# mike-gimelfarb/bboptpy

Measured on AMD Instinct MI355X. Metric: candidate-evals/sec, higher is better.
Workload: dtype f64; 1 GPU; ActiveCMAES n=128 np=4096 rosenbrock, 256 independent populations per GPU in lockstep; populations_per_gpu=256, n=128, np=4096, objective=rosenbrock

## Files before the change

bboptpy_amd/csrc/bbo_cma.hip:

```cpp
#include "bbo_cma_kernels.hpp"
#include "bbo_sep_kernels.hpp"
#include "bbo_chol_kernels.hpp"
#include "bbo_eig_mw.hpp"

#include <algorithm>
#include <atomic>
#include <cmath>
#include <cstdlib>
#include <limits>

namespace bbo {

namespace {

enum { K_SAMPLE = 0, K_RANK, K_WHITEN, K_GRAM, K_PATHS, K_COV, K_EIGEN, K_POST, K_STOP, K_COUNT };
static const char *const K_NAMES[K_COUNT] = { "bbo:cma_sample_eval", "bbo:cma_rank", "bbo:cma_whiten", "bbo:cma_gram", "bbo:cma_paths", "bbo:cma_cov", "bbo:cma_eigen", "bbo:cma_post", "bbo:cma_history_stop" };

int pick_maxt(int ld)
{
    const int per_wave = ((ld >> 4) + 3) / 4;
    if (per_wave <= 1) return 1;
    if (per_wave <= 2) return 2;
    if (per_wave <= 4) return 4;
    return 8;
// ... 381 lines not shown
}

void CmaEngine::launch_post(int mode)
{
    const CmaConst &c = c_;
    if (c.ld <= 128) {
        const size_t lds = (size_t) (c.ld * (c.ld + 2) + c.ld) * sizeof(double);
        allow_lds((const void*) cma_post_mfma<1>, 140 * 1024);
        allow_lds((const void*) cma_post_mfma<4>, 140 * 1024);
        if (c.npop < 32)
            hipLaunchKernelGGL(cma_post_mfma<4>, dim3(c.npop, 4), dim3(256), lds, stream_, d_, c_,
                    mode);
        else
            hipLaunchKernelGGL(cma_post_mfma<1>, dim3(c.npop, 1), dim3(256), lds, stream_, d_, c_,
                    mode);
    } else {
        dim3 grid(c.ld / 16, c.ld / 16, c.npop);
        hipLaunchKernelGGL(cma_post, grid, dim3(256), 0, stream_, d_, c_, mode);
    }
}

SampleRoute CmaEngine::sample_route() const
{
    const CmaConst &c = c_;
    SampleRoute r {};
    r.gy = c.npop;
    r.writes_zn = c.variant != 2;
    auto is = [&r](SampleKernel k, int gx, int block, size_t lds) {
        r.k = k;
        r.gx = gx;
        r.block = block;
        r.lds = lds;
    };
    if (c.variant == 2) {
        const int per_pop = std::max(1, 4096 / c.npop);
        if (c.ld <= 256)
            is(SK_SEP_16, std::min((c.lambda_pad + 15) / 16, per_pop), 256, (size_t) 16 * c.ld * sizeof(double));
        else if (c.ld <= 2048) {
            is(SK_SEP_64_512, std::min((c.lambda_pad + 7) / 8, per_pop), 512, (size_t) 8 * c.ld * sizeof(double));
            r.full = nothing_to_guard() ? 1 : 0;
            if (r.full && sep_sum_objective(c.obj) && !(d_.dbg & DBG_SEP_ROWS_LDS))
                is(c.ld == 1024 && c.obj != OBJ_RASTRIGIN && c.obj != OBJ_DIFFPOW ? SK_SEP_SUM4 : SK_SEP_SUM,
                        std::min(c.lambda_pad / (4 * SEP_K), per_pop), 256, 0);
            else if (r.full)
                r.k = SK_SEP_64_512_LEAN;
        } else
            is(SK_SEP_64, std::min((c.lambda_pad + 3) / 4, per_pop), 256, (size_t) 4 * c.ld * sizeof(double));
    } else if (c.ld == 128 && (long) c.npop * c.lambda_pad >= sample128_min_rows_
            && (c.obj < 0 || frag_objective_ok(c.obj))) {
        r.rows_per_wg = rows_per_workgroup((long) c.npop * c.lambda_pad, 4096);
        is(c.variant == 3 && chol_tri_ ? SK_EVAL128_TRI : SK_EVAL128, (c.lambda_pad + r.rows_per_wg - 1) / r.rows_per_wg,
                512, 128 * 1024);
        r.full = nothing_to_guard() ? 1 : 0;
    } else if (c.ld == 128 && (long) c.npop * (c.lambda_pad / 16) <= sample_wide_max_tiles_)
        is(c.variant == 3 && chol_tri_ ? SK_TILE8_TRI : SK_TILE8, c.lambda_pad / 16, 512,
                (size_t) 16 * (c.ld + 2) * sizeof(double));
    else if (c.ld <= 128)
        is(c.ld <= 32 ? SK_EVAL64_1_8 : c.ld <= 64 ? SK_EVAL64_1 : SK_EVAL64_2, (c.lambda_pad + 63) / 64, 256,
                (size_t) 64 * (c.ld + 2) * sizeof(double));
    else {
        const int tiles = c.lambda_pad / 16;
        const size_t lds = (size_t) 16 * (c.ld + 2) * sizeof(double);
        if ((long) tiles * c.npop <= 32 && c.ld <= 256 && !(d_.dbg & DBG_SAMPLE_4WAVES))
            is(SK_TILE16, tiles, 1024, lds);
        else
            is(pick_maxt(c.ld) == 4 ? SK_EVAL_4 : SK_EVAL_8, tiles, 256, lds);
    }
    return r;
}

void CmaEngine::launch_sample_eval()
{
    const SampleRoute r = sample_route();
    auto go = [&](auto kernel, int allow, auto... args) {
        if (allow) allow_lds((const void*) kernel, allow);
        hipLaunchKernelGGL(kernel, dim3(r.gx, r.gy), dim3(r.block), r.lds, stream_, d_, c_, args...);
    };
    timer_.begin(stream_, K_SAMPLE);
    switch (r.k) {
    case SK_NONE: break;
    case SK_SEP_16: go(sep_sample_eval<16>, 128 * 1024); break;
    case SK_SEP_64_512: go(sep_sample_eval<64, 512>, 140 * 1024); break;
    case SK_SEP_64_512_LEAN: go(sep_sample_eval<64, 512, true>, 140 * 1024); break;
    case SK_SEP_SUM: go(sep_sum_kernel<0>(c_.obj), 0); break;
    case SK_SEP_SUM4: go(sep_sum_kernel<4>(c_.obj), 0); break;
    case SK_SEP_64: go(sep_sample_eval<64>, 140 * 1024); break;
    case SK_EVAL128: go(cma_sample_eval128, 128 * 1024, r.rows_per_wg, r.full); break;
    case SK_EVAL128_TRI: go(cma_sample_eval128_tri, 128 * 1024, r.rows_per_wg, r.full); break;
    case SK_TILE8: go(cma_sample_eval<1, 8>, 0); break;
    case SK_TILE8_TRI: go(cma_sample_eval<1, 8, true>, 0); break;
    case SK_EVAL64_1_8: go(cma_sample_eval64<1, 8>, 0); break;
    case SK_EVAL64_1: go(cma_sample_eval64<1>, 80 * 1024); break;
    case SK_EVAL64_2: go(cma_sample_eval64<2>, 80 * 1024); break;
    case SK_TILE16: go(cma_sample_eval<1, 16>, 0); break;
    case SK_EVAL_4: go(cma_sample_eval<4>, 0); break;
    case SK_EVAL_8: go(cma_sample_eval<8>, 80 * 1024); break;
    }
    timer_.end(stream_);
    BBO_HIP(hipGetLastError());
    c_.use_zn = (r.writes_zn && !c_.bound) ? 1 : 0;
    last_sample_ = r;
}

void CmaEngine::launch_rank()
{
    const CmaConst &c = c_;
    rank_wrote_norms_ = false;
    timer_.begin(stream_, K_RANK);
    last_rank_ = rank_route(c.lambda, c.npop, d_.dbg);
    switch (last_rank_) {
    case RK_WAVE:
        hipLaunchKernelGGL(cma_rank_wave, dim3((c.npop + 3) / 4), dim3(256), 0, stream_, d_, c_);
        break;
    case RK_COUNT64:
        hipLaunchKernelGGL(cma_rank64, dim3((c.lambda + 3) / 4, c.npop), dim3(256), 0, stream_, d_, c_);
        break;
    case RK_COUNT32:
        hipLaunchKernelGGL(cma_rank32, dim3((c.lambda + 7) / 8, c.npop), dim3(256), 0, stream_, d_, c_);
        break;
    case RK_COUNT8:
        hipLaunchKernelGGL(cma_rank, dim3((c.lambda + 31) / 32, c.npop), dim3(256), 0, stream_, d_, c_);
        break;
    default: {
        const int m = rank_sort_m(c.lambda);
        allow_lds((const void*) cma_rank_sort, 128 * 1024);
        const size_t lds = rank_sort_merges(m, d_.dbg) ? (size_t) m * 24 : (size_t) std::max(m, 1024) * 12;
        hipLaunchKernelGGL(cma_rank_sort, dim3(c.npop), dim3(sort_threads(m)), lds, stream_, d_,
                c_, m);
        break;
    }
    }
    if (last_rank_ != RK_WAVE) rank_wrote_norms_ = c.variant == 1 && c.use_zn && !basis_maybe_stale_;
    timer_.end(stream_);
    BBO_HIP(hipGetLastError());
}

UpdateRoute CmaEngine::update_route(bool norms_done, bool with_cov) const
{
    const CmaConst &c = c_;
    UpdateRoute r {};
    auto add = [&r](UpdateKernel k, int slot, int gx, int gy, int gz, int block, size_t lds = 0, int arg = 0) {
// ... 488 lines not shown
    if (k == "C") return o.rows(C_, p * ld, c.n, c.n, c.ld);
    if (k == "invsqrtC") {
        if (c.lazy_isc && out) {
            const int hs = c_.honor_stop;
            c_.honor_stop = 0;
            launch_post(3);
            c_.honor_stop = hs;
            BBO_HIP(hipGetLastError());
            BBO_HIP(hipStreamSynchronize(stream_));
        }
        return o.rows(isc_, p * ld, c.n, c.n, c.ld);
    }
    if (k == "BD") {
        if (out && cap >= (int) (n * n)) {
            std::vector<double> pk(ld * ld);
            BDp_.download(pk.data(), ld * ld, p * ld * ld);
            for (size_t i = 0; i < n; i++)
                for (size_t j = 0; j < n; j++) out[i * n + j] = pk[bfrag_index(i, j, ld)];
        }
        return (int) (n * n);
    }
    if (k == "arx") return o.rows(X_, (size_t) p * c.lambda_pad, c.lambda, c.n, c.ld);
    if (k == "weights") {
        if (out && cap >= c.mu) weights_.download(out, c.mu);
        return c.mu;
    }
    if (k == "fitness") {
        if (out && cap >= c.lambda) f_.download(out, c.lambda, (size_t) p * c.lambda_pad);
        return c.lambda;
    }
    if (k == "fit_idx" || k == "fit_val" || k == "rank") {
        if (out && cap >= c.lambda) {
            std::vector<int> ord(c.lambda);
            (k == "rank" ? rank_ : order_).download(ord.data(), c.lambda,
                    (size_t) p * c.lambda_pad);
            if (k == "fit_val") {
                std::vector<double> f(c.lambda);
                f_.download(f.data(), c.lambda, (size_t) p * c.lambda_pad);
                for (int i = 0; i < c.lambda; i++) out[i] = f[ord[i]];
            } else {
                for (int i = 0; i < c.lambda; i++) out[i] = ord[i];
            }
        }
        return c.lambda;
    }
    if (k == "ycoeff") {
        if (out && cap >= c.mu) {
            std::vector<double> S(c.mu_pad);
            S_.download(S.data(), c.mu_pad, (size_t) p * c.mu_pad);
            for (int i = 0; i < c.mu; i++) out[i] = S[i] / std::max(S[c.mu - 1 - i], 1e-8);
        }
        return c.mu;
    }
    if (k == "zlast") {
        const size_t cnt = (size_t) c.lambda * n;
        if (!zrecord_.p) return 0;
        if (out && cap >= (int) cnt) zrecord_.download(out, cnt, p * cnt);
        return (int) cnt;
    }
    if (k == "profile") return profile_report(out, cap);
    if (const int r = prog_get(k, out, cap); r >= 0) return r;
    if (k == "eig_work") {
        const size_t cnt = std::min((size_t) 4 * eig_slab(c.ld), eig_work_.count);
        if (out && (size_t) cap >= cnt) eig_work_.download(out, cnt, (size_t) p * 4 * eig_slab(c.ld));
        return (int) cnt;
    }
    if (k == "eig_stamps") {
        if (!stamps_.p) return 0;
        if (out && cap >= 48) {
            long long t[48];
            stamps_.download(t, 48);
            for (int i = 0; i < 48; i++) out[i] = (double) t[i];
        }
        return 48;
    }
    if (k == "best_hist" || k == "kth_hist") {
        if (out && cap >= c.hlen)
            (k == "best_hist" ? hist_best_ : hist_kth_).download(out, c.hlen, (size_t) p * c.hlen);
        return c.hlen;
    }
    CmaScal s;
    scal_.download(&s, 1, p);
    if (k == "sigma") return o.one(s.sigma);
    if (k == "it") return o.one(s.it);
    if (k == "fev") return o.one(s.fev);
    if (k == "flag") return o.one(s.flag);
    if (k == "stop") return o.one(s.stop);
    if (k == "hsig") return o.one(s.hsig);
    if (k == "pslen") return o.one(s.pslen);
    if (k == "fbest") return o.one(s.fbest);
    if (k == "fworst") return o.one(s.fworst);
    if (k == "eigenlastev") return o.one(s.eigenlastev);
    if (k == "eigen_done") return o.one(s.eigen_done);
    if (k == "basis_ok") return o.one(s.basis_ok);
    if (k == "eig_stage") return o.one(s.eig_stage);
    if (k == "eig_mw_fail") return o.one(s.eig_mw_fail);
    if (k == "chol_repairs") {
        if (c.variant != 3) throw Error(BBO_ERR_KEY, "'chol_repairs' belongs to CholeskyCMAES");
        int r = 0;
        chol_repairs_.download(&r, 1, p);
        return o.one(r);
    }
    if (c.variant == 3 && k == "chol_tri") return o.one(chol_tri_ ? 1 : 0);
    if (c.variant == 3 && k == "stol") return o.one(c.stol);
    if (c.variant == 3 && k == "ranked") return o.one(c.ranked);
    if (k == "eig_mw_off") return o.one(mw_disabled_ ? 1 : 0);
    if (k == "eig_split_maxp") return o.one(split_maxp_);
    if (k == "eig_fixed128") return o.one(last_route_.fixed ? 1 : 0);
    if (k == "cov_fused") return o.one(last_route_.forms_c ? 1 : 0);
    if (k == "eig_route") {
        double ids[sizeof(last_route_.step) / sizeof(last_route_.step[0])];
        for (int i = 0; i < last_route_.count; i++) ids[i] = last_route_.step[i].k;
        return o.copy(ids, last_route_.count);
    }
    if (k == "rank_route") return o.one(last_rank_);
    if (k == "sample_route") return o.one(last_sample_.k);
    if (k == "sample_lean") return o.one(last_sample_.full);
    if (k == "update_route") {
        double ids[sizeof(last_update_.step) / sizeof(last_update_.step[0])];
        for (int i = 0; i < last_update_.count; i++) ids[i] = last_update_.step[i].k;
        return o.copy(ids, last_update_.count);
    }
    if (k == "small_fused") return o.one(small_fused_ ? 1 : 0);
    if (k == "splits") return o.one(c.splits);
    if (k == "gram_coef_stamp") {
        int stamp = 0;
        if (coef_stamp_.p) coef_stamp_.download(&stamp, 1, p);
        return o.one(stamp);
    }
    if (k == "eig_mw_reserved") return o.one((double) mw_reserved_);
    if (k == "eig_mw_capacity") {
        MwBudget &b = MwBudget::get();
        std::lock_guard<std::mutex> lock(b.m);
        return o.one((double) b.capacity(params_.device));
    }
    if (k == "best_len") return o.one(s.hist_len);
    if (k == "best_buffer") return o.one(s.hist_head);
    if (k == "ibest") return o.one(s.ibw[0]);
    if (k == "ybw") return o.copy(s.ybw, 4);
    if (k == "ibw") {
        const double ids[4] = { (double) s.ibw[0], (double) s.ibw[1], (double) s.ibw[2], (double) s.ibw[3] };
        return o.copy(ids, 4);
    }
    if (k == "n") return o.one(c.n);
    if (k == "lambda") return o.one(c.lambda);
    if (k == "mu") return o.one(c.mu);
    if (k == "mueff") return o.one(c.mueff);
    if (k == "cc") return o.one(c.cc);
    if (k == "cs") return o.one(c.cs);
    if (k == "c1") return o.one(c.c1);
    if (k == "cmu") return o.one(c.cmu);
    if (k == "cneg") return o.one(c.cneg);
    if (k == "alphaold") return o.one(c.alphaold);
    if (k == "cm") return o.one(c.cm);
    if (k == "ccov") return o.one(c.ccov);
    if (k == "damps") return o.one(c.damps);
    if (k == "chi") return o.one(c.chi);
    if (k == "eigenfreq") return o.one(c.eigenfreq);
    if (k == "hlen") return o.one(c.hlen);
    if (k == "ik") return o.one(c.ik);
    if (k == "mit") return o.one(c.mit);
    if (k == "mfev") return o.one(c.mfev);
    if (k == "sigma0") return o.one(c.sigma0);
    throw Error(BBO_ERR_KEY, "unknown state key '" + k + "'");
}

int CmaEngine::set(const std::string &k, int p, const double *in, int count)
{
    enter_population("set()", p);
    rank_wrote_norms_ = false;
// ... 41 lines not shown
        f_.upload(f.data(), c.lambda, (size_t) p * c.lambda_pad);
        return count;
    }
    if (k == "xmean") return vec_in(xmean_);
    if (k == "xold") return vec_in(xold_);
    if (k == "pc") return vec_in(pc_);
    if (k == "ps") return vec_in(ps_);
    if (k == "csep") {
        BBO_REQUIRE(c.variant == 2, "csep belongs to SepCMAES");
        const int r = vec_in(csep_);
        std::vector<double> dd(ld, 1.);
        for (size_t i = 0; i < n; i++) dd[i] = std::sqrt(in[i]);
        D_.upload(dd.data(), ld, p * ld);
        return r;
    }
    if (k == "C") return mat_in(C_);
    if (k == "best_hist" || k == "kth_hist") {
        BBO_REQUIRE(count == c.hlen, "set: wrong element count");
        (k == "best_hist" ? hist_best_ : hist_kth_).upload(in, c.hlen, (size_t) p * c.hlen);
        return count;
    }
    if (k == "invsqrtC") throw Error(BBO_ERR_KEY, "invsqrtC is derived from B and D: set those");
    if (k == "B" || k == "D") {
        int r;
        if (k == "D") {
            BBO_REQUIRE(count == (int) n, "set: wrong element count");
            std::vector<double> tmp(ld, 1.);
            std::copy(in, in + n, tmp.begin());
            D_.upload(tmp.data(), ld, p * ld);
            r = count;
        } else {
            r = mat_in(B_);
        }
        c_.honor_stop = 0;
        launch_post(1);
        BBO_HIP(hipGetLastError());
        BBO_HIP(hipStreamSynchronize(stream_));
        return r;
    }
    if (k == "profile") return profile_enable(in, K_COUNT, K_NAMES);
    if (const int r = prog_set(k, in, count); r >= 0) return r;
    if (k == "dbg") {
        d_.dbg = (int) in[0];
        return 1;
    }
    if (c.variant == 3 && k == "chol_tri") {
        chol_tri_ = in[0] != 0.;
        return 1;
    }
    if (k == "sample_wide_max") {
        sample_wide_max_tiles_ = (long) in[0];
        return 1;
    }
    if (k == "sample128_min") {
        sample128_min_rows_ = (long) in[0];
        return 1;
    }
    if (k == "eig_split_maxp") {
        split_maxp_ = (int) in[0];
        return 1;
    }
    if (k == "stop_off") {
        c_.stop_off = (int) in[0];
        return 1;
    }
    if (k == "ftarget") {
        c_.ftarget = in[0];
        return 1;
    }
    if (k == "eig_stamps") {
        if (stamps_.count != 48) stamps_.alloc(48);
        BBO_HIP(hipStreamSynchronize(stream_));
        BBO_HIP(hipMemset(stamps_.p, 0, 48 * sizeof(long long)));
        d_.stamps = stamps_.p;
        return 1;
    }
    if (k == "record_normals") {
        BBO_REQUIRE(count == 1, "set: wrong element count");
        if (in[0] != 0.) {
            const size_t want = (size_t) c.npop * c.lambda * n;
            if (zrecord_.count != want) zrecord_.alloc(want);
            d_.zrecord = zrecord_.p;
        } else {
            d_.zrecord = nullptr;
        }
        return 1;
    }
    BBO_REQUIRE(count == 1, "set: wrong element count");
    CmaScal s;
    scal_.download(&s, 1, p);
    if (k == "sigma") s.sigma = in[0];
    else if (k == "it") s.it = (int) in[0];
    else if (k == "fev") s.fev = (int) in[0];
    else if (k == "eigenlastev") s.eigenlastev = (int) in[0];
    else if (k == "fbest") s.fbest = in[0];
    else if (k == "fworst") s.fworst = in[0];
    else if (k == "stop") s.stop = (int) in[0];
    else if (k == "best_len") s.hist_len = (int) in[0];
    else if (k == "best_buffer") s.hist_head = (int) in[0];
    else throw Error(BBO_ERR_KEY, "unknown state key '" + k + "'");
    scal_.upload(&s, 1, p);
    return 1;
}

size_t eigen_view_scratch(int ld)
{
// ... 19 lines not shown
```

bboptpy_amd/csrc/bbo_cma.hpp:

```cpp
#pragma once

#include "bbo_engine.hpp"

namespace bbo {

struct CmaScal {
    double sigma;
    double fbest, fworst;
    double pslen;
    double ybw[4];
    int ibw[4];
    int it, fev;
    int flag;
    int stop;
    int hsig;
    int eigenlastev, eigen_done;
    int hist_head, hist_len;
    int basis_ok;
    int eig_stage;
    int eig_mw_fail;
};

struct CmaConst {
    int n, ld;
// ... 76 lines not shown
    double *mean_part;
    double *hist_best, *hist_kth;
    double *eig_work;
    const double *weights;
    const double *lower, *upper, *aux;
    const double *zinject;
    double *zrecord;
    CmaScal *scal;
    long long *stamps;
    int dbg;
    int mw_fault;
    int *mw_fail_host;
};

enum EigKernel : int {
    EK_EIGEN_SMALL = 0, EK_EIGEN_128, EK_EIGEN_256, EK_EIGEN, EK_EIGEN_FX128, EK_EIGEN_FX128U,
    EK_EIGEN_R1, EK_EIGEN_R1_FX128, EK_EIGEN_G1, EK_TRED_MW, EK_TRED_TAIL, EK_EIG_HALVES,
    EK_EIGEN_G2, EK_EIG_SECULAR, EK_EIG_LOWNER, EK_EIG_FCOLS, EK_EIGEN_G,
    EK_TRED_MW512, EK_TRED_MW_CHAIN, EK_EIGEN_B4, EK_EIGEN_B,
    EK_EIG_GEMM1, EK_EIG_GEMM, EK_EIG_WY4, EK_EIG_WY4_512, EK_EIG_WY,
    EK_POST, EK_POST_MFMA
};

struct EigRoute {
    struct Step {
        EigKernel k;
        int arg;
    };
    Step step[12];
    int count;
    int timed;
    bool split;
    bool post;
    bool fixed;
    bool forms_c;
    long mw_workgroups;
};

enum SampleKernel : int {
    SK_NONE = -1,
    SK_SEP_16 = 0, SK_SEP_64_512, SK_SEP_64_512_LEAN, SK_SEP_SUM, SK_SEP_SUM4, SK_SEP_64,
    SK_EVAL128, SK_EVAL128_TRI, SK_TILE8, SK_TILE8_TRI,
    SK_EVAL64_1_8, SK_EVAL64_1, SK_EVAL64_2,
    SK_TILE16, SK_EVAL_4, SK_EVAL_8
};

struct SampleRoute {
    SampleKernel k;
    int gx, gy, block;
    size_t lds;
    int rows_per_wg;
    int full;
    bool writes_zn;
};

enum UpdateKernel : int {
    UK_CHOL_PATHS = 0, UK_CHOL_CPRIME, UK_CHOL_FACTOR, UK_SEP_MOMENTS, UK_SEP_PATHS,
    UK_WHITEN128, UK_WHITEN, UK_GRAM128S, UK_GRAM128, UK_GRAM,
    UK_PATHS, UK_PATHS_LAZY, UK_PATHS_LAZY1K, UK_COV
};

struct UpdateRoute {
    struct Step {
        UpdateKernel k;
        int slot;
        int gx, gy, gz, block;
        size_t lds;
        int arg;
    };
    Step step[4];
    int count;
};

class CmaEngine: public Engine<CmaScal> {
public:
    static constexpr const char *HANDLE_NAME = "not a CMA-ES handle";
    explicit CmaEngine(const bbo_params &p);
    ~CmaEngine() override;

    void init(int n, const double *lower, const double *upper, const double *guess,
            const ObjectiveSpec &obj) override;
    void solution(int population, double *x_out, int *n_evals, int *converged) override;
    void optimize(int n, const double *lower, const double *upper, const double *guess,
            const ObjectiveSpec &obj, double *x_out, int *n_evals, int *converged) override;
    int get(const std::string &key, int population, double *out, int cap) override;
    int set(const std::string &key, int population, const double *in, int count) override;
    int dimension() const override { return c_.n; }

    void set_params(int np, double sigma, int mfev);
    void phase(int which);
    void inject_normals(const double *z, int count);
    double evaluate_point(const double *x);
    int lambda() const { return params_.np; }
    int populations() const { return params_.populations; }
    uint64_t seed() const { return params_.seed; }
    void set_seed(uint64_t s) { params_.seed = s; }
    void fresh_start(uint64_t s)
    {
        params_.seed = s;
        keep_bc_ = false;
    }

private:
    static const bbo_params &checked(const bbo_params &p);
    void generation(bool honor_stop) override;
    bool budget_spent(const CmaScal &s) const override { return s.fev >= c_.mfev; }
    void inspect(const std::vector<CmaScal> &sc) override;
    int chunk_limit(int want) override;
    void launch_chunk(int gens) override;
    void after_chunk(bool in_run) override;
    bool small_fused_ok() const;
    void launch_small(int gens, bool honor_stop);
    void launch_sample_eval();
    void launch_post(int mode);
    void launch_rank();
    void launch_update(bool with_cov = true);
    SampleRoute sample_route() const;
    UpdateRoute update_route(bool norms_done, bool with_cov) const;
    EigRoute eig_route(bool spread_ok = true, bool fuse_ok = false) const;
    void launch_eigen(EigRoute r);
    bool nothing_to_guard() const
    {
        return c_.n == c_.ld && !c_.bound && c_.lambda == c_.lambda_pad && !d_.zinject && !d_.zrecord
                && !(d_.dbg & DBG_SAMPLE_GUARDED);
    }
    void launch_history_stop();
    void host_evaluate();
    void program_evaluate();

    CmaConst c_ {};
    CmaDev d_ {};
    bool keep_bc_ = false;
    bool basis_maybe_stale_ = false;
    DevBuf<double> mw_buf_;
    unsigned long long mw_launch_ = 0;
    bool mw_disabled_ = false;
    int mw_xcd_ = next_mw_xcd();
    static int next_mw_xcd();
    long sample_wide_max_tiles_ = 512;
    long sample128_min_rows_ = 256 * 128;
    bool chol_tri_ = true;
    int split_maxp_ = 32;
    EigRoute last_route_ {};
    SampleRoute last_sample_ { SK_NONE };
    UpdateRoute last_update_ {};
    bool small_fused_ = false;
    int last_rank_ = -1;
    bool rank_wrote_norms_ = false;
    int last_n_ = -1;

    DevBuf<double> zn2_, csep_, A_;
    DevBuf<double> X_, f_, xmean_, xold_, pc_, ps_, C_, B_, D_, isc_, BDp_, ISp_, S_,
            gram_part_, mean_part_, hist_best_, hist_kth_, eig_work_, weights_, zinject_, zrecord_;
    DevBuf<double> coef_tab_;
    DevBuf<int> rank_, order_, chol_repairs_, coef_stamp_;
    void coef_tab_forget();
    DevBuf<long long> stamps_;
    int *mw_fail_host_ = nullptr;
    long mw_reserved_ = 0;
    bool mw_launched_ = false;
    bool mw_reserve(long workgroups);
    void mw_release();
    bool mw_check_failed();
};

}
```

bboptpy_amd/csrc/bbo_cma_kernels.hpp:

```cpp
#pragma once

#include "bbo_cma.hpp"
#include "bbo_objectives.hpp"
#include "bbo_rng.hpp"
#include "bbo_eig.hpp"
#include "bbo_rank.hpp"

namespace bbo {

typedef double d4_t __attribute__((ext_vector_type(4)));

#define BBO_INF (__builtin_huge_val())

__device__ inline void cma_draw_quad(const CmaDev &d, const CmaConst &c, int p, int row, int q,
        int gen, uint32_t sw, const double2 *tab, double (&z)[4])
{
    const int j0 = cma_quad_col0(q);
    z[0] = z[1] = z[2] = z[3] = 0.;
    if (row < c.lambda && j0 < c.n) {
        if (d.zinject) {
            const double *zi = d.zinject + ((size_t) p * c.lambda + row) * c.n;
#pragma unroll
            for (int i = 0; i < 4; i++)
                if (j0 + 4 * i < c.n) z[i] = zi[j0 + 4 * i];
// ... 284 lines not shown
                d.f[(size_t) p * c.lambda_pad + row] = f;
            }
        }
    }
}

template<int MAXT, int KSM = 32>
__global__ __launch_bounds__(256) void cma_sample_eval64(CmaDev d, CmaConst c)
{
    extern __shared__ __attribute__((aligned(16))) double lds[];
    sample_eval64_body<MAXT, KSM>(d, c, blockIdx.y, blockIdx.x, lds, blockIdx.y);
}

template<bool FULL>
__device__ inline void sample128_epilogue(const CmaDev &d, const CmaConst &c, int p, int rowbase,
        double sigma, const d4_t (&acc)[8], int lane, const double *xm)
{
    const int fr = lane & 15, fk = lane >> 4;
    const int n = FULL ? 128 : c.n;
    double *Xp = d.X + (size_t) p * c.lambda_pad * 128 + ((size_t) rowbase + fk) * 128 + fr;
    double x[8][4];
#pragma unroll
    for (int t = 0; t < 8; t++) {
        const int col = t * 16 + fr;
        const double xmc = xm[col];
#pragma unroll
        for (int r = 0; r < 4; r++) {
            double v = 0.;
            if (FULL) {
                v = xmc + sigma * acc[t][r];
            } else if (col < n) {
                v = xmc + sigma * acc[t][r];
                if (c.bound) v = fmax(d.lower[col], fmin(v, d.upper[col]));
            }
            x[t][r] = v;
            Xp[(size_t) (4 * r) * 128 + t * 16] = v;
        }
    }
    if (c.obj >= 0) {
        double f[4];
        eval_frag_rows<8>(c.obj, n, x, d.aux, lane, f);
        if (fr == 0) {
#pragma unroll
            for (int r = 0; r < 4; r++) {
                const int rr = rowbase + fk + 4 * r;
                double fv = f[r];
                if ((!FULL && !(rr < c.lambda)) || fv != fv) fv = BBO_INF;
                d.f[(size_t) p * c.lambda_pad + rr] = fv;
            }
        }
    }
}

template<bool FULL, bool TRI = false>
__device__ __forceinline__ void sample_eval128_body(const CmaDev &d, const CmaConst &c,
        int rows_per_wg, double *bd, const double2 *ntab, const double *ftab, const double *xms)
{
    const int p = blockIdx.y, row0 = blockIdx.x * rows_per_wg;
    const CmaScal *sc = d.scal + p;
    const int tid = threadIdx.x, lane = tid & 63, wave = tid >> 6;
    const int gen = sc->it;
    const double sigma = sc->sigma;
    const int tiles = min(rows_per_wg, c.lambda_pad - row0) >> 4;
    const int fr = lane & 15, fk = lane >> 4;
    const uint32_t sw = stream_word(STREAM_CMA_NORMAL, (uint32_t) p);

    for (int tile = wave; tile < tiles; tile += 8) {
        const int rowbase = row0 + tile * 16;
        const int row = rowbase + fr;
        d4_t acc[8];
#pragma unroll
        for (int t = 0; t < 8; t++) acc[t] = d4_t { 0., 0., 0., 0. };
        double zz = 0.;
        if (FULL) {
            double z[32];
            uint32_t pend = normal_quads_fast<8>(c.seed, (uint32_t) row, (uint32_t) fk, 4u,
                    (uint32_t) gen, sw, ntab, z);
            while (pend) {
                const int b = __ffs(pend) - 1;
                pend &= pend - 1;
                const double v = normal_quad_settle(c.seed, (uint32_t) row,
                        (uint32_t) (4 * (b >> 2) + fk), (uint32_t) (b & 3), (uint32_t) gen, sw,
                        ntab, ftab);
#pragma unroll
                for (int i = 0; i < 32; i++) z[i] = (i == b) ? v : z[i];
            }
#pragma unroll
            for (int i = 0; i < 32; i++) zz = __builtin_fma(z[i], z[i], zz);
            int hi = lane + 8192;
            asm volatile("" : "+v"(hi));
            auto frag = [&](int i, int t) {
                const int idx = (i >> 3) * 8 + t * 32 + (i & 7);
                return idx < 128 ? bd[lane + idx * 64] : bd[hi + (idx - 128) * 64];
            };
            double pre[8];
#pragma unroll
            for (int t = 0; t < 8; t++) pre[t] = frag(0, t);
#pragma unroll
            for (int i = 0; i < 32; i++) {
#pragma unroll
                for (int t = 0; t < 8; t++) {
                    if (TRI && (i >> 2) > t) continue;
                    const double bv = (i & 3) == 0 ? pre[t] : frag(i, t);
                    acc[t] = __builtin_amdgcn_mfma_f64_16x16x4f64(z[i], bv, acc[t], 0, 0, 0);
                }
                if ((i & 3) == 3) {
                    if (i + 1 < 32) {
#pragma unroll
                        for (int t = 0; t < 8; t++)
                            if (!TRI || ((i + 1) >> 2) <= t) pre[t] = frag(i + 1, t);
                    }
                    __builtin_amdgcn_sched_barrier(0);
                }
            }
        } else {
#pragma unroll 1
            for (int kc = 0; kc < 4; kc++) {
                double a[8];
#pragma unroll
                for (int h = 0; h < 2; h++) {
                    double z[4];
                    cma_draw_quad(d, c, p, row, 4 * (2 * kc + h) + fk, gen, sw, ntab, z);
#pragma unroll
                    for (int i = 0; i < 4; i++) {
                        a[4 * h + i] = z[i];
                        zz = __builtin_fma(z[i], z[i], zz);
                    }
                }
                const double *bk = bd + kc * 8 * 64 + lane;
#pragma unroll
                for (int i = 0; i < 8; i++) {
#pragma unroll
                    for (int t = 0; t < 8; t++) {
                        if (TRI && 2 * kc + (i >> 2) > t) continue;
                        acc[t] = __builtin_amdgcn_mfma_f64_16x16x4f64(a[i], bk[(t * 32 + i) * 64],
                                acc[t], 0, 0, 0);
                    }
                }
            }
        }
        zz += __shfl_xor(zz, 16, 64);
        zz += __shfl_xor(zz, 32, 64);
        if (fk == 0) d.zn2[(size_t) p * c.lambda_pad + row] = zz;
        sample128_epilogue<FULL>(d, c, p, rowbase, sigma, acc, lane, xms);
    }
}

__global__ __launch_bounds__(512, 1) void cma_sample_eval128(CmaDev d, CmaConst c, int rows_per_wg,
        int full)
{
    const int p = blockIdx.y;
    const CmaScal *sc = d.scal + p;
    if (pop_frozen(c, sc)) return;
    extern __shared__ __attribute__((aligned(16))) double bd[];
    const int tid = threadIdx.x;
    {
        const double2 *src = reinterpret_cast<const double2*>(d.BDp + (size_t) p * 128 * 128);
        double2 *dst = reinterpret_cast<double2*>(bd);
#pragma unroll
        for (int i = 0; i < 16; i++) dst[tid + 512 * i] = src[tid + 512 * i];
    }
    __shared__ double2 ntab[NORMAL_TABLE_N];
    __shared__ double ftab[NORMAL_FTABLE_N];
    __shared__ double xms[128];
    normal_table_fill(ntab, tid, 512);
    normal_ftable_fill(ftab, tid, 512);
    if (tid < 128) xms[tid] = d.xmean[(size_t) p * 128 + tid];
    __syncthreads();
    if (full) sample_eval128_body<true>(d, c, rows_per_wg, bd, ntab, ftab, xms);
    else sample_eval128_body<false>(d, c, rows_per_wg, bd, ntab, ftab, xms);
}

__global__ __launch_bounds__(512, 1) void cma_sample_eval128_tri(CmaDev d, CmaConst c, int rows_per_wg,
        int full)
{
    const int p = blockIdx.y;
    const CmaScal *sc = d.scal + p;
    if (pop_frozen(c, sc)) return;
    extern __shared__ __attribute__((aligned(16))) double bd[];
    const int tid = threadIdx.x;
    {
        const double2 *src = reinterpret_cast<const double2*>(d.BDp + (size_t) p * 128 * 128);
        double2 *dst = reinterpret_cast<double2*>(bd);
#pragma unroll
        for (int i = 0; i < 16; i++) dst[tid + 512 * i] = src[tid + 512 * i];
    }
    __shared__ double2 ntab[NORMAL_TABLE_N];
    __shared__ double ftab[NORMAL_FTABLE_N];
    __shared__ double xms[128];
    normal_table_fill(ntab, tid, 512);
    normal_ftable_fill(ftab, tid, 512);
    if (tid < 128) xms[tid] = d.xmean[(size_t) p * 128 + tid];
    __syncthreads();
    if (full) sample_eval128_body<true, true>(d, c, rows_per_wg, bd, ntab, ftab, xms);
    else sample_eval128_body<false, true>(d, c, rows_per_wg, bd, ntab, ftab, xms);
}

template<int SL>
__device__ __forceinline__ void cma_rank_body(const CmaDev &d, const CmaConst &c)
{
    const int p = blockIdx.y;
    CmaScal *sc = d.scal + p;
    if (pop_frozen(c, sc)) return;
    __shared__ __attribute__((aligned(16))) double tile[RANK_TILE];
    const int tid = threadIdx.x;
    const int cand = blockIdx.x * (256 / SL) + tid / SL, slice = tid % SL;
    const double *f = d.f + (size_t) p * c.lambda_pad;
    const bool live = cand < c.lambda;
    const int cnt = rank_by_counting<SL>(f, c.lambda, cand, slice, tile);
    const bool norms = c.variant == 1 && c.use_zn && sc->basis_ok;
    if (live && slice == 0) {
        const double fi = f[cand];
        d.rank[(size_t) p * c.lambda_pad + cand] = cnt;
        d.order[(size_t) p * c.lambda_pad + cnt] = cand;
        if (cnt == 0) { sc->ibw[0] = cand; sc->ybw[0] = fi; }
        if (cnt == 1) { sc->ibw[1] = cand; sc->ybw[1] = fi; }
        if (cnt == c.lambda - 2) { sc->ibw[2] = cand; sc->ybw[2] = fi; }
        if (cnt == c.lambda - 1) { sc->ibw[3] = cand; sc->ybw[3] = fi; }
        if (norms && cnt >= c.lambda - c.mu)
            d.S[(size_t) p * c.mu_pad + cnt - (c.lambda - c.mu)] =
                    sc->sigma * sc->sigma * d.zn2[(size_t) p * c.lambda_pad + cand];
    }
    if (norms && blockIdx.x == 0)
        for (int wr = c.mu + tid; wr < c.mu_pad; wr += 256) d.S[(size_t) p * c.mu_pad + wr] = 0.;
    if (blockIdx.x == 0 && tid == 0) sc->fev += c.lambda;
}

__global__ __launch_bounds__(256) void cma_rank(CmaDev d, CmaConst c)
{
    cma_rank_body<8>(d, c);
}
__global__ __launch_bounds__(256) void cma_rank32(CmaDev d, CmaConst c)
{
    cma_rank_body<32>(d, c);
}
__global__ __launch_bounds__(256) void cma_rank64(CmaDev d, CmaConst c)
{
    cma_rank_body<64>(d, c);
}

constexpr int G128_CH = 32;
__host__ __device__ constexpr int coef_tab_chunks(int lambda_pad) { return (lambda_pad + G128_CH - 1) / G128_CH; }

static_assert((int) DBG_RANK_COUNT32 == RANK_DBG_COUNT32 && (int) DBG_RANK_COUNT_NO64 == RANK_DBG_COUNT_NO64
        && (int) DBG_RANK_BITONIC == RANK_DBG_BITONIC, "bbo_rank.hpp reads these bits of CmaDev::dbg");

__global__ __launch_bounds__(1024) void cma_rank_sort(CmaDev d, CmaConst c, int m)
// ... 1452 lines not shown
```

bboptpy_amd/csrc/bbo_objectives.hpp:

```cpp
#pragma once

#include <hip/hip_runtime.h>

#include "bbo_wave.hpp"

namespace bbo {

enum Objective : int {
    OBJ_HOST = -1,
    OBJ_SPHERE = 0,
    OBJ_ROSENBROCK = 1,
    OBJ_RASTRIGIN = 2,
    OBJ_ELLIPSOID = 3,
    OBJ_ACKLEY = 4,
    OBJ_GRIEWANK = 5,
    OBJ_CIGAR = 6,
    OBJ_DISCUS = 7,
    OBJ_DIFFPOW = 8,
    OBJ_SCHWEFEL12 = 9,
    OBJ_COUNT = 10
};

constexpr double TWO_PI = 6.283185307179586476925286766559;
constexpr double EULER_E = 2.718281828459045235360287471352;
// ... 162 lines not shown
        switch (obj) {
        case OBJ_SPHERE:
#pragma unroll
            for (int t = 0; t < NT; t++) a += (16 * t + c0 < n) ? x[t][r] * x[t][r] : 0.;
            f[r] = row16_sum(a);
            break;
        case OBJ_ROSENBROCK:
#pragma unroll
            for (int t = 0; t < NT; t++) {
                const double xj = x[t][r];
                const double xn = row16_next(c0 == 0 ? x[t + 1 < NT ? t + 1 : t][r] : xj);
                const double tt = xn - xj * xj;
                const double u = 1. - xj;
                a += (16 * t + c0 + 1 < n) ? 100. * (tt * tt) + u * u : 0.;
            }
            f[r] = row16_sum(a);
            break;
        case OBJ_ELLIPSOID:
#pragma unroll
            for (int t = 0; t < NT; t++)
                a += (16 * t + c0 < n) ? aux[16 * t + c0] * (x[t][r] * x[t][r]) : 0.;
            f[r] = row16_sum(a);
            break;
        case OBJ_CIGAR:
        case OBJ_DISCUS: {
#pragma unroll
            for (int t = 0; t < NT; t++) {
                const int j = 16 * t + c0;
                a += (j > 0 && j < n) ? x[t][r] * x[t][r] : 0.;
            }
            a = row16_sum(a);
            const double x0 = row16_sum(c0 == 0 ? x[0][r] : 0.);
            f[r] = obj == OBJ_CIGAR ? x0 * x0 + 1.0e6 * a : 1.0e6 * (x0 * x0) + a;
            break;
        }
        case OBJ_SCHWEFEL12: {
            double carry = 0.;
#pragma unroll
            for (int t = 0; t < NT; t++) {
                const double v = (16 * t + c0 < n) ? x[t][r] : 0.;
                const double run = carry + row16_scan(v);
                a += (16 * t + c0 < n) ? run * run : 0.;
                carry += row16_sum(v);
            }
            f[r] = row16_sum(a);
            break;
        }
        default:
            f[r] = 0.;
        }
    }
}

}
```

bboptpy_amd/csrc/bbo_wave.hpp:

```cpp
#pragma once

#include <hip/hip_runtime.h>

namespace bbo {

__device__ inline void wave_sync()
{
    __builtin_amdgcn_fence(__ATOMIC_SEQ_CST, "wavefront");
    __builtin_amdgcn_wave_barrier();
}

template<class C, class S>
__device__ inline bool pop_frozen(const C &c, const S *sc)
{
    return c.honor_stop && sc->stop != 0;
}

template<int CTRL>
__device__ inline int dpp_mov(int v)
{
    return __builtin_amdgcn_mov_dpp(v, CTRL, 0xf, 0xf, true);
}

template<int CTRL>
__device__ inline double dpp_mov(double v)
{
    const int lo = dpp_mov<CTRL>(__double2loint(v)), hi = dpp_mov<CTRL>(__double2hiint(v));
    return __hiloint2double(hi, lo);
}

template<int G>
__device__ inline double group_sum(double v)
{
#pragma unroll
    for (int off = G / 2; off > 0; off >>= 1) v += __shfl_xor(v, off, G);
    return v;
}

template<int G>
__device__ inline double group_prod(double v)
{
#pragma unroll
    for (int off = G / 2; off > 0; off >>= 1) v *= __shfl_xor(v, off, G);
    return v;
}

__device__ inline void wave_argmin(double &v, int &s)
{
#pragma unroll
    for (int off = 32; off > 0; off >>= 1) {
        const double ov = __shfl_xor(v, off, 64);
        const int os = __shfl_xor(s, off, 64);
        if (ov < v || (ov == v && os < s)) {
            v = ov;
            s = os;
        }
    }
}
__device__ inline void wave_argmax(double &v, int &s)
{
#pragma unroll
    for (int off = 32; off > 0; off >>= 1) {
        const double ov = __shfl_xor(v, off, 64);
        const int os = __shfl_xor(s, off, 64);
        if (ov > v || (ov == v && os < s)) {
            v = ov;
            s = os;
        }
    }
}

template<int NW>
__device__ inline double block_sum(double v, double *scratch)
{
    const int tid = threadIdx.x;
    v = group_sum<64>(v);
    __syncthreads();
    if ((tid & 63) == 0) scratch[tid >> 6] = v;
    __syncthreads();
    double s = scratch[0];
// ... 40 lines not shown
```

Baseline: 731.9 million candidate-evals/s.

## Transpose MFMA output tile in 128-dim sampler so each lane holds contiguous columns

Adds a transposed path for the 128-dimension sample/eval kernel. The BD matrix is stored in LDS permuted, and the MFMA operands are swapped so each lane holds four contiguous coordinates of one row. Stores become vectorized double2 writes and the objective is evaluated per lane with only two cross-lane reductions; Rosenbrock's neighbour term uses a bpermute. The aim is to cut the scattered epilogue stores and the row-reduction shuffles, at the cost of a strided LDS fill and an extra code path for selected objectives.

```diff
diff --git a/bboptpy_amd/csrc/bbo_cma.hip b/bboptpy_amd/csrc/bbo_cma.hip
--- a/bboptpy_amd/csrc/bbo_cma.hip
+++ b/bboptpy_amd/csrc/bbo_cma.hip
@@ -457,6 +457,7 @@
         is(c.variant == 3 && chol_tri_ ? SK_EVAL128_TRI : SK_EVAL128, (c.lambda_pad + r.rows_per_wg - 1) / r.rows_per_wg,
                 512, 128 * 1024);
         r.full = nothing_to_guard() ? 1 : 0;
+        r.transposed = r.full && !sample128_rowlayout_ && (c.obj < 0 || frag_cols_objective_ok(c.obj)) ? 1 : 0;
     } else if (c.ld == 128 && (long) c.npop * (c.lambda_pad / 16) <= sample_wide_max_tiles_)
         is(c.variant == 3 && chol_tri_ ? SK_TILE8_TRI : SK_TILE8, c.lambda_pad / 16, 512,
                 (size_t) 16 * (c.ld + 2) * sizeof(double));
@@ -490,8 +491,8 @@
     case SK_SEP_SUM: go(sep_sum_kernel<0>(c_.obj), 0); break;
     case SK_SEP_SUM4: go(sep_sum_kernel<4>(c_.obj), 0); break;
     case SK_SEP_64: go(sep_sample_eval<64>, 140 * 1024); break;
-    case SK_EVAL128: go(cma_sample_eval128, 128 * 1024, r.rows_per_wg, r.full); break;
-    case SK_EVAL128_TRI: go(cma_sample_eval128_tri, 128 * 1024, r.rows_per_wg, r.full); break;
+    case SK_EVAL128: go(cma_sample_eval128, 128 * 1024, r.rows_per_wg, r.full, r.transposed); break;
+    case SK_EVAL128_TRI: go(cma_sample_eval128_tri, 128 * 1024, r.rows_per_wg, r.full, r.transposed); break;
     case SK_TILE8: go(cma_sample_eval<1, 8>, 0); break;
     case SK_TILE8_TRI: go(cma_sample_eval<1, 8, true>, 0); break;
     case SK_EVAL64_1_8: go(cma_sample_eval64<1, 8>, 0); break;
@@ -1086,6 +1087,16 @@
         }
         return c.mu;
     }
+    if (k == "S") {
+        if (c.variant != 1) throw Error(BBO_ERR_KEY, "'S' belongs to ActiveCMAES");
+        if (out && cap >= c.mu) S_.download(out, c.mu, (size_t) p * c.mu_pad);
+        return c.mu;
+    }
+    if (k == "zn2") {
+        if (!zn2_.p) return 0;
+        if (out && cap >= c.lambda) zn2_.download(out, c.lambda, (size_t) p * c.lambda_pad);
+        return c.lambda;
+    }
     if (k == "zlast") {
         const size_t cnt = (size_t) c.lambda * n;
         if (!zrecord_.p) return 0;
@@ -1150,6 +1161,8 @@
     if (k == "rank_route") return o.one(last_rank_);
     if (k == "sample_route") return o.one(last_sample_.k);
     if (k == "sample_lean") return o.one(last_sample_.full);
+    if (k == "sample_transposed") return o.one(last_sample_.transposed);
+    if (k == "sample128_rowlayout") return o.one(sample128_rowlayout_ ? 1 : 0);
     if (k == "update_route") {
         double ids[sizeof(last_update_.step) / sizeof(last_update_.step[0])];
         for (int i = 0; i < last_update_.count; i++) ids[i] = last_update_.step[i].k;
@@ -1297,6 +1310,10 @@
         sample_wide_max_tiles_ = (long) in[0];
         return 1;
     }
+    if (k == "sample128_rowlayout") {
+        sample128_rowlayout_ = in[0] != 0.;
+        return 1;
+    }
     if (k == "sample128_min") {
         sample128_min_rows_ = (long) in[0];
         return 1;
diff --git a/bboptpy_amd/csrc/bbo_cma.hpp b/bboptpy_amd/csrc/bbo_cma.hpp
--- a/bboptpy_amd/csrc/bbo_cma.hpp
+++ b/bboptpy_amd/csrc/bbo_cma.hpp
@@ -152,6 +152,7 @@
     int rows_per_wg;
     int full;
     bool writes_zn;
+    int transposed;
 };
 
 enum UpdateKernel : int {
@@ -240,6 +241,7 @@
     long sample_wide_max_tiles_ = 512;
     long sample128_min_rows_ = 256 * 128;
     bool chol_tri_ = true;
+    bool sample128_rowlayout_ = false;
     int split_maxp_ = 32;
     EigRoute last_route_ {};
     SampleRoute last_sample_ { SK_NONE };
diff --git a/bboptpy_amd/csrc/bbo_cma_kernels.hpp b/bboptpy_amd/csrc/bbo_cma_kernels.hpp
--- a/bboptpy_amd/csrc/bbo_cma_kernels.hpp
+++ b/bboptpy_amd/csrc/bbo_cma_kernels.hpp
@@ -360,10 +360,57 @@
     }
 }
 
-template<bool FULL, bool TRI = false>
+__device__ inline void sample128_epilogue_tr(const CmaDev &d, const CmaConst &c, int p, int rowbase,
+        double sigma, const d4_t (&acc)[8], int lane, const double *xm)
+{
+    const int fr = lane & 15, fk = lane >> 4;
+    const size_t row = (size_t) p * c.lambda_pad + rowbase + fr;
+    double2 *Xp = reinterpret_cast<double2*>(d.X + row * 128 + 4 * fk);
+    const double2 *xm2 = reinterpret_cast<const double2*>(xm + 4 * fk);
+    double x[8][4];
+#pragma unroll
+    for (int t = 0; t < 8; t++) {
+        const double2 m0 = xm2[8 * t], m1 = xm2[8 * t + 1];
+        x[t][0] = m0.x + sigma * acc[t][0];
+        x[t][1] = m0.y + sigma * acc[t][1];
+        x[t][2] = m1.x + sigma * acc[t][2];
+        x[t][3] = m1.y + sigma * acc[t][3];
+        Xp[8 * t] = double2 { x[t][0], x[t][1] };
+        Xp[8 * t + 1] = double2 { x[t][2], x[t][3] };
+    }
+    if (c.obj >= 0) {
+        double fv = eval_frag_cols<8>(c.obj, x, d.aux, lane);
+        if (fk == 0) {
+            if (fv != fv) fv = BBO_INF;
+            d.f[row] = fv;
+        }
+    }
+}
+
+__device__ inline void sample128_fill(double *bd, const double *bdp, int tid, int transposed)
+{
+    const double2 *src = reinterpret_cast<const double2*>(bdp);
+    if (transposed) {
+#pragma unroll
+        for (int i = 0; i < 16; i++) {
+            const int e = 2 * (tid + 512 * i), m = e & 15;
+            const double2 v = src[tid + 512 * i];
+            double *dst = bd + (e & ~15) + 4 * (m & 3) + (m >> 2);
+            dst[0] = v.x;
+            dst[4] = v.y;
+        }
+    } else {
+        double2 *dst = reinterpret_cast<double2*>(bd);
+#pragma unroll
+        for (int i = 0; i < 16; i++) dst[tid + 512 * i] = src[tid + 512 * i];
+    }
+}
+
+template<bool FULL, bool TRI = false, bool TR = false>
 __device__ __forceinline__ void sample_eval128_body(const CmaDev &d, const CmaConst &c,
         int rows_per_wg, double *bd, const double2 *ntab, const double *ftab, const double *xms)
 {
+    static_assert(FULL || !TR, "the transposed tile has no masked form");
     const int p = blockIdx.y, row0 = blockIdx.x * rows_per_wg;
     const CmaScal *sc = d.scal + p;
     const int tid = threadIdx.x, lane = tid & 63, wave = tid >> 6;
@@ -410,7 +457,8 @@
                 for (int t = 0; t < 8; t++) {
                     if (TRI && (i >> 2) > t) continue;
                     const double bv = (i & 3) == 0 ? pre[t] : frag(i, t);
-                    acc[t] = __builtin_amdgcn_mfma_f64_16x16x4f64(z[i], bv, acc[t], 0, 0, 0);
+                    acc[t] = TR ? __builtin_amdgcn_mfma_f64_16x16x4f64(bv, z[i], acc[t], 0, 0, 0)
+                                : __builtin_amdgcn_mfma_f64_16x16x4f64(z[i], bv, acc[t], 0, 0, 0);
                 }
                 if ((i & 3) == 3) {
                     if (i + 1 < 32) {
@@ -450,57 +498,50 @@
         zz += __shfl_xor(zz, 16, 64);
         zz += __shfl_xor(zz, 32, 64);
         if (fk == 0) d.zn2[(size_t) p * c.lambda_pad + row] = zz;
-        sample128_epilogue<FULL>(d, c, p, rowbase, sigma, acc, lane, xms);
+        if (TR) sample128_epilogue_tr(d, c, p, rowbase, sigma, acc, lane, xms);
+        else sample128_epilogue<FULL>(d, c, p, rowbase, sigma, acc, lane, xms);
     }
 }
 
 __global__ __launch_bounds__(512, 1) void cma_sample_eval128(CmaDev d, CmaConst c, int rows_per_wg,
-        int full)
+        int full, int transposed)
 {
     const int p = blockIdx.y;
     const CmaScal *sc = d.scal + p;
     if (pop_frozen(c, sc)) return;
     extern __shared__ __attribute__((aligned(16))) double bd[];
     const int tid = threadIdx.x;
-    {
-        const double2 *src = reinterpret_cast<const double2*>(d.BDp + (size_t) p * 128 * 128);
-        double2 *dst = reinterpret_cast<double2*>(bd);
-#pragma unroll
-        for (int i = 0; i < 16; i++) dst[tid + 512 * i] = src[tid + 512 * i];
-    }
+    sample128_fill(bd, d.BDp + (size_t) p * 128 * 128, tid, transposed);
     __shared__ double2 ntab[NORMAL_TABLE_N];
     __shared__ double ftab[NORMAL_FTABLE_N];
-    __shared__ double xms[128];
+    __shared__ __attribute__((aligned(16))) double xms[128];
     normal_table_fill(ntab, tid, 512);
     normal_ftable_fill(ftab, tid, 512);
     if (tid < 128) xms[tid] = d.xmean[(size_t) p * 128 + tid];
     __syncthreads();
-    if (full) sample_eval128_body<true>(d, c, rows_per_wg, bd, ntab, ftab, xms);
+    if (transposed) sample_eval128_body<true, false, true>(d, c, rows_per_wg, bd, ntab, ftab, xms);
+    else if (full) sample_eval128_body<true>(d, c, rows_per_wg, bd, ntab, ftab, xms);
     else sample_eval128_body<false>(d, c, rows_per_wg, bd, ntab, ftab, xms);
 }
 
 __global__ __launch_bounds__(512, 1) void cma_sample_eval128_tri(CmaDev d, CmaConst c, int rows_per_wg,
-        int full)
+        int full, int transposed)
 {
     const int p = blockIdx.y;
     const CmaScal *sc = d.scal + p;
     if (pop_frozen(c, sc)) return;
     extern __shared__ __attribute__((aligned(16))) double bd[];
     const int tid = threadIdx.x;
-    {
-        const double2 *src = reinterpret_cast<const double2*>(d.BDp + (size_t) p * 128 * 128);
-        double2 *dst = reinterpret_cast<double2*>(bd);
-#pragma unroll
-        for (int i = 0; i < 16; i++) dst[tid + 512 * i] = src[tid + 512 * i];
-    }
+    sample128_fill(bd, d.BDp + (size_t) p * 128 * 128, tid, transposed);
     __shared__ double2 ntab[NORMAL_TABLE_N];
     __shared__ double ftab[NORMAL_FTABLE_N];
-    __shared__ double xms[128];
+    __shared__ __attribute__((aligned(16))) double xms[128];
     normal_table_fill(ntab, tid, 512);
     normal_ftable_fill(ftab, tid, 512);
     if (tid < 128) xms[tid] = d.xmean[(size_t) p * 128 + tid];
     __syncthreads();
-    if (full) sample_eval128_body<true, true>(d, c, rows_per_wg, bd, ntab, ftab, xms);
+    if (transposed) sample_eval128_body<true, true, true>(d, c, rows_per_wg, bd, ntab, ftab, xms);
+    else if (full) sample_eval128_body<true, true>(d, c, rows_per_wg, bd, ntab, ftab, xms);
     else sample_eval128_body<false, true>(d, c, rows_per_wg, bd, ntab, ftab, xms);
 }
 
diff --git a/bboptpy_amd/csrc/bbo_objectives.hpp b/bboptpy_amd/csrc/bbo_objectives.hpp
--- a/bboptpy_amd/csrc/bbo_objectives.hpp
+++ b/bboptpy_amd/csrc/bbo_objectives.hpp
@@ -238,4 +238,74 @@
     }
 }
 
-}
+__host__ __device__ inline bool frag_cols_objective_ok(int obj)
+{
+    return obj == OBJ_SPHERE || obj == OBJ_ROSENBROCK || obj == OBJ_ELLIPSOID || obj == OBJ_CIGAR
+            || obj == OBJ_DISCUS;
+}
+
+template<int NT>
+__device__ inline double eval_frag_cols(int obj, const double (&x)[NT][4], const double *aux, int lane)
+{
+    const int fk = lane >> 4;
+    double a[4] = { 0., 0., 0., 0. };
+    switch (obj) {
+    case OBJ_SPHERE:
+#pragma unroll
+        for (int t = 0; t < NT; t++)
+#pragma unroll
+            for (int r = 0; r < 4; r++) a[r] += x[t][r] * x[t][r];
+        break;
+    case OBJ_ROSENBROCK: {
+        const int up = ((lane + 16) & 63) << 2;
+#pragma unroll
+        for (int t = 0; t < NT; t++) {
+            const double xn3 = lane_read64(fk == 0 ? x[t + 1 < NT ? t + 1 : t][0] : x[t][0], up);
+#pragma unroll
+            for (int r = 0; r < 4; r++) {
+                const double xj = x[t][r];
+                const double xn = r < 3 ? x[t][r < 3 ? r + 1 : r] : xn3;
+                const double tt = xn - xj * xj;
+                const double u = 1. - xj;
+                const double term = 100. * (tt * tt) + u * u;
+                a[r] += (t == NT - 1 && r == 3 && fk == 3) ? 0. : term;
+            }
+        }
+        break;
+    }
+    case OBJ_ELLIPSOID: {
+        const double *w = aux + 4 * fk;
+#pragma unroll
+        for (int t = 0; t < NT; t++)
+#pragma unroll
+            for (int r = 0; r < 4; r++) a[r] += w[16 * t + r] * (x[t][r] * x[t][r]);
+        break;
+    }
+    case OBJ_CIGAR:
+    case OBJ_DISCUS:
+#pragma unroll
+        for (int t = 0; t < NT; t++)
+#pragma unroll
+            for (int r = 0; r < 4; r++) {
+                const double sq = x[t][r] * x[t][r];
+                a[r] += (t == 0 && r == 0 && fk == 0) ? 0. : sq;
+            }
+        break;
+    default:
+        return 0.;
+    }
+    double q[4];
+#pragma unroll
+    for (int r = 0; r < 4; r++) {
+        const double s = a[r] + __shfl_xor(a[r], 32, 64);
+        q[r] = s + __shfl_xor(s, 16, 64);
+    }
+    const double f = (q[0] + q[2]) + (q[1] + q[3]);
+    if (obj == OBJ_CIGAR || obj == OBJ_DISCUS) {
+        const double x0 = x[0][0];
+        return obj == OBJ_CIGAR ? x0 * x0 + 1.0e6 * f : 1.0e6 * (x0 * x0) + f;
+    }
+    return f;
+}
+
+}
diff --git a/bboptpy_amd/csrc/bbo_wave.hpp b/bboptpy_amd/csrc/bbo_wave.hpp
--- a/bboptpy_amd/csrc/bbo_wave.hpp
+++ b/bboptpy_amd/csrc/bbo_wave.hpp
@@ -26,6 +26,13 @@
 __device__ inline double dpp_mov(double v)
 {
     const int lo = dpp_mov<CTRL>(__double2loint(v)), hi = dpp_mov<CTRL>(__double2hiint(v));
+    return __hiloint2double(hi, lo);
+}
+
+__device__ inline double lane_read64(double v, int byte)
+{
+    const int lo = __builtin_amdgcn_ds_bpermute(byte, __double2loint(v));
+    const int hi = __builtin_amdgcn_ds_bpermute(byte, __double2hiint(v));
     return __hiloint2double(hi, lo);
 }
 
```

Result: faster. 740.3 million candidate-evals/s (median of 6 runs) (+1.1%).
